# prstrive/SCGaussian

Hardware: AMD Instinct MI355X
Metric: train_iters_per_sec (higher is better)
Workload: dtype f32; 1 GPU; S2: 200000 Gaussians, 1008x756, SH degree 3, fwd+bwd per view (BASELINE configs[1] shape: LLFF-fern 3-view training, 200 k Gaussians @ 1008x756); gaussians=200000, width=1008, height=756, sh_degree=3, visible=174771, views=3, parallelism=single, ranks_seen=1, launched_by=single process, grad_bucket_bytes=0, grad_bucket_bytes_per_view=0

## Files before the change

scgaussian_amd/csrc/blend.hip:

```cpp
#include "scg_common.h"
#include "tile_sort.h"

namespace scg {

constexpr float kHalfLog2e = 0.72134752044448170f;
typedef float f32x2 __attribute__((ext_vector_type(2)));
typedef float f32x4 __attribute__((ext_vector_type(4)));

__device__ __forceinline__ bool splat_hits_rect(const float4& a, const float4& b, float x0, float y0) {
    const float dx0 = x0 - a.x, dy0 = y0 - a.y, dx1 = dx0 + 7.0f, dy1 = dy0 + 7.0f;
    const float nx = __builtin_amdgcn_fmed3f(0.0f, dx0, dx1), ny = __builtin_amdgcn_fmed3f(0.0f, dy0, dy1);
    const float cb2 = a.w + a.w;
    const float ya = __builtin_amdgcn_fmed3f(b.w * nx, dy0, dy1);
    const float qa = nx * (a.z * nx + cb2 * ya) + b.x * ya * ya;
    const float xb = __builtin_amdgcn_fmed3f(-a.w * ny * __builtin_amdgcn_rcpf(a.z), dx0, dx1);
    const float qb = ny * (b.x * ny + cb2 * xb) + a.z * xb * xb;
    return !((qa > b.z) && (qb > b.z));
}

__device__ __forceinline__ int quadrant_workgroup(int wg, int n_tiles, const uint2* __restrict__ ranges, int& quad) {
    quad = (wg >> 3) & 3;
    const int per = (n_tiles + 7) >> 3;
    const uint32_t* order = reinterpret_cast<const uint32_t*>(ranges) + 2 * (size_t)n_tiles;
    return (int)order[(wg & 7) * per + (wg >> 5)];
}

__device__ __forceinline__ void wave_sync() {
    __builtin_amdgcn_fence(__ATOMIC_ACQ_REL, "wavefront");
    __builtin_amdgcn_wave_barrier();
}

typedef const uint32_t __attribute__((address_space(3))) * LdsIds;
template <class IdList>
__device__ __forceinline__ void forward_walk(float4* s_rec, const FrameDev& f, int tile, int quad, int lane, uint2 range,
                                             IdList list,
                                             const float4* __restrict__ splats, float* __restrict__ out_color,
                                             float* __restrict__ out_depth, float* __restrict__ out_alpha,
                                             float* __restrict__ final_T, uint32_t* __restrict__ n_contrib) {
    const int tile_x = tile % f.gx, tile_y = tile / f.gx;
    const int qx0 = tile_x * kTile + (quad & 1) * 8, qy0 = tile_y * kTile + (quad >> 1) * 8;
    const int px = qx0 + (lane & 7), py = qy0 + (lane >> 3);
    const bool inside = (px < f.W) && (py < f.H);
    const float pxf = (float)px, pyf = (float)py;

    const int n = (int)(range.y - range.x);
    float T = inside ? 1.0f : -1.0f;
    int bgi0 = __builtin_amdgcn_readfirstlane(__builtin_bit_cast(int, f.bg[0]));
    int bgi1 = __builtin_amdgcn_readfirstlane(__builtin_bit_cast(int, f.bg[1]));
    int bgi2 = __builtin_amdgcn_readfirstlane(__builtin_bit_cast(int, f.bg[2]));
    asm volatile("" : "+s"(bgi0), "+s"(bgi1), "+s"(bgi2));
    f32x2 Crg = {0.f, 0.f}, Cbz = {0.f, 0.f};
    uint32_t last = 0;
    int n_blended = 0;
#ifndef SCG_FWD_TRIP_CXX
    const uint32_t lds_base = (uint32_t)reinterpret_cast<uintptr_t>(s_rec);
    const uint64_t exec_all = __builtin_amdgcn_read_exec();
#endif

    uint32_t id_next = 0;
    float4 ra, rb, rc;
    if (n > 0) {
        const uint32_t id0 = list[min(lane, n - 1)];
        id_next = list[min(kWave + lane, n - 1)];
        ra = splats[3 * (size_t)id0 + 0]; rb = splats[3 * (size_t)id0 + 1]; rc = splats[3 * (size_t)id0 + 2];
    }

    for (int base = 0; base < n; base += kWave) {
        if (__all(T < 0.0f)) break;
        const bool hit = (base + lane < n) && splat_hits_rect(ra, rb, (float)qx0, (float)qy0);
        if (hit) {
            *reinterpret_cast<float2*>(&s_rec[2 * kWave + lane]) = make_float2(ra.x, ra.y);
            s_rec[kWave + lane] = make_float4(kHalfLog2e * ra.z, 2.0f * kHalfLog2e * ra.w, kHalfLog2e * rb.x, rb.y);
            s_rec[lane] = rc;
        }
        uint64_t m = __ballot(hit);
        if (base + kWave < n) {
            ra = splats[3 * (size_t)id_next + 0]; rb = splats[3 * (size_t)id_next + 1];
            rc = splats[3 * (size_t)id_next + 2];
            id_next = list[min(base + 2 * kWave + lane, n - 1)];
        }
        wave_sync();

        n_blended += __builtin_popcountll(m);
#ifdef SCG_FWD_TRIP_CXX
        while (m) {
            const int j = __builtin_ctzll(m);
            asm("s_bitset0_b64 %0, %1" : "+s"(m) : "s"(j));
            const float2 c = *reinterpret_cast<const float2*>(&s_rec[2 * kWave + j]);
            const float4 q = s_rec[kWave + j];
            const float dx = c.x - pxf, dy = c.y - pyf;
            const float u = __builtin_fmaf(q.y, dy, q.x * dx);
            const float t = __builtin_fmaf(u, dx, (q.z * dy) * dy);
            const float alpha = fminf(kAlphaMax, q.w * __builtin_amdgcn_exp2f(-t));
            const float wgt = T * alpha;
            const float test_T = __builtin_fmaf(-T, alpha, T);
            if ((t >= 0.0f) && (alpha >= kAlphaMin)) {
                const bool contributes = test_T >= kTEps;
                const float T_prev = T;
                T = contributes ? test_T : -fabsf(T_prev);
                if (contributes) {
                    const float4 col = s_rec[j];
                    const f32x2 ww = {wgt, wgt};
                    Crg = __builtin_elementwise_fma((f32x2){col.x, col.y}, ww, Crg);
                    Cbz = __builtin_elementwise_fma((f32x2){col.z, col.w}, ww, Cbz);
                    last = (uint32_t)(base + j + 1);
                }
            }
        }
#else
        int last_j = -1;
        while (m) {
            const int j = __builtin_ctzll(m);
            asm("s_bitset0_b64 %0, %1" : "+s"(m) : "s"(j));
            asm volatile(
                "v_lshl_add_u32 v63, %[j], 4, %[lds]\n\t"
                "ds_read_b64 v[48:49], v63 offset:2048\n\t"
                "ds_read_b128 v[52:55], v63 offset:1024\n\t"
                "s_waitcnt lgkmcnt(1)\n\t"
                "v_sub_f32_e32 v48, v48, %[px]\n\t"
                "v_sub_f32_e32 v49, v49, %[py]\n\t"
                "s_waitcnt lgkmcnt(0)\n\t"
                "v_mul_f32_e32 v58, v52, v48\n\t"
                "v_mul_f32_e32 v59, v54, v49\n\t"
                "v_fmac_f32_e32 v58, v53, v49\n\t"
                "v_mul_f32_e32 v60, v59, v49\n\t"
                "v_fmac_f32_e32 v60, v58, v48\n\t"
                "v_exp_f32_e64 v56, -v60\n\t"
                "v_cmpx_le_f32_e32 vcc, 0, v60\n\t"
                "v_mul_f32_e32 v56, v55, v56\n\t"
                "v_min_f32_e32 v56, 0x3f7d70a4, v56\n\t"
                "v_cmpx_le_f32_e32 vcc, %[amin], v56\n\t"
                "v_fma_f32 v57, -%[T], v56, %[T]\n\t"
                "v_mul_f32_e32 v56, %[T], v56\n\t"
                "v_or_b32_e32 %[T], 0x80000000, %[T]\n\t"
                "v_cmpx_le_f32_e32 vcc, %[eps], v57\n\t"
                "v_mov_b32_e32 %[T], v57\n\t"
                "ds_read_b128 v[44:47], v63\n\t"
                "v_mov_b32_e32 %[lj], %[j]\n\t"
                "s_waitcnt lgkmcnt(0)\n\t"
                "v_pk_fma_f32 %[crg], v[44:45], v[56:57], %[crg] op_sel_hi:[1,0,1]\n\t"
                "v_pk_fma_f32 %[cbz], v[46:47], v[56:57], %[cbz] op_sel_hi:[1,0,1]\n\t"
                "s_mov_b64 exec, %[all]"
                : [T] "+v"(T), [crg] "+v"(Crg), [cbz] "+v"(Cbz), [lj] "+v"(last_j)
                : [j] "s"(j), [lds] "v"(lds_base), [px] "v"(pxf), [py] "v"(pyf), [amin] "s"(kAlphaMin), [eps] "s"(kTEps),
                  [all] "s"(exec_all)
                : "memory", "vcc", "v44", "v45", "v46", "v47", "v48", "v49", "v52", "v53", "v54", "v55", "v56", "v57", "v58",
                  "v59", "v60", "v63");
        }
        if (last_j >= 0) last = (uint32_t)(base + last_j + 1);
#endif
        wave_sync();
    }

    if (f.cost_out && lane == 0) atomicMax(f.cost_out + tile, (uint32_t)n_blended);
    if (inside) {
        T = fabsf(T);
        const size_t pix = (size_t)py * f.W + px;
        const size_t hw = (size_t)f.H * f.W;
        out_color[pix] = Crg[0] + T * __builtin_bit_cast(float, bgi0);
        out_color[hw + pix] = Crg[1] + T * __builtin_bit_cast(float, bgi1);
        out_color[2 * hw + pix] = Cbz[0] + T * __builtin_bit_cast(float, bgi2);
        out_depth[pix] = Cbz[1];
        out_alpha[pix] = 1.0f - T;
        if (final_T) final_T[pix] = T;
        if (n_contrib) n_contrib[pix] = last;
    }
}


__global__ __launch_bounds__(kWave) void blend_forward_kernel(FrameDev f, const uint2* __restrict__ ranges,
                                                              const uint32_t* __restrict__ point_list,
                                                              const float4* __restrict__ splats,
                                                              float* __restrict__ out_color,
                                                              float* __restrict__ out_depth,
                                                              float* __restrict__ out_alpha,
                                                              float* __restrict__ final_T,
                                                              uint32_t* __restrict__ n_contrib,
                                                              float4* __restrict__ zero_fill, uint32_t zero_vec) {
    __shared__ float4 s_rec[3 * kWave];
    if (zero_fill) {
        for (uint32_t i = blockIdx.x * kWave + threadIdx.x; i < zero_vec; i += gridDim.x * kWave)
            zero_fill[i] = make_float4(0.f, 0.f, 0.f, 0.f);
    }

    const int n_tiles = f.gx * f.gy;
    int quad;
    const int tile = quadrant_workgroup(blockIdx.x, n_tiles, ranges, quad);
    if (tile >= n_tiles) return;
    const uint2 range = ranges[tile];
    forward_walk(s_rec, f, tile, quad, (int)threadIdx.x, range, point_list + range.x, splats, out_color, out_depth, out_alpha,
                 final_T, n_contrib);
}

template <int NW>
__device__ __forceinline__ void fused_long_list_fallback(unsigned char* smem, const uint32_t* __restrict__ depth_keys,
                                                      uint32_t* __restrict__ list, int n, uint64_t* __restrict__ keys,
                                                      uint64_t* __restrict__ keys2) {
    if (!sort_long_list<NW * kWave, kFusedLongBuckets, 2>(smem, depth_keys, list, n, keys, keys2)) {
        __syncthreads();
        for (int i = threadIdx.x; i < n; i += NW * kWave) {
            const uint32_t id = list[i];
            keys[i] = ((uint64_t)depth_keys[id] << 32) | (uint64_t)id;
        }
        __syncthreads();
        bitonic_sort_asc(keys, n, true);
        __syncthreads();
        for (int i = threadIdx.x; i < n; i += NW * kWave) list[i] = (uint32_t)keys[i];
    }
}

template <int MAX_N, int CNT, int WPE, int NW = 4>
__global__ __launch_bounds__(NW * kWave) __attribute__((amdgpu_waves_per_eu(WPE, WPE))) void tile_blend_forward_kernel(
    FrameDev f, const uint2* __restrict__ ranges, uint32_t* __restrict__ point_list,
    const uint32_t* __restrict__ depth_keys, int id_bits, const float4* __restrict__ splats,
    float* __restrict__ out_color, float* __restrict__ out_depth, float* __restrict__ out_alpha,
    float* __restrict__ final_T, uint32_t* __restrict__ n_contrib, float4* __restrict__ zero_fill, uint32_t zero_vec,
    uint64_t* __restrict__ spill, uint64_t* __restrict__ spill2, const uint32_t* __restrict__ class_counts,
    int long_presorted) {
    typedef TileSortLds<NW, MAX_N, CNT> Lds;
    constexpr size_t kIdsBytes = sizeof(uint32_t) * MAX_N, kPlanesBytes = 4 * 3 * kWave * sizeof(float4);
    constexpr size_t kLdsBytes = sizeof(Lds) > kIdsBytes + kPlanesBytes ? sizeof(Lds) : kIdsBytes + kPlanesBytes;
    __shared__ __attribute__((aligned(16))) unsigned char smem[kLdsBytes];
    Lds& L = *reinterpret_cast<Lds*>(smem);
    static_assert(offsetof(Lds, id) == 0, "the sorted ids lie in front of the record planes");
    static_assert(kLdsBytes >= (2 * kFusedLongBuckets + 4 + 2 * 4) * sizeof(uint32_t), "the fallback's counters must fit");
    if (zero_fill) {
        for (uint32_t i = blockIdx.x * blockDim.x + threadIdx.x; i < zero_vec; i += gridDim.x * blockDim.x)
            zero_fill[i] = make_float4(0.f, 0.f, 0.f, 0.f);
    }
    if (f.long_out && blockIdx.x == 0 && threadIdx.x == 0) {
        f.long_out[0] = class_counts[0] + class_counts[1];
        f.long_out[1] = class_counts[3];
    }
    const int n_tiles = f.gx * f.gy, per = (n_tiles + 7) >> 3;
    const uint32_t* order = reinterpret_cast<const uint32_t*>(ranges) + 2 * (size_t)n_tiles;
    const int tile = (int)order[(blockIdx.x & 7) * per + (blockIdx.x >> 3)];
    if (tile >= n_tiles) return;
    const uint2 range = ranges[tile];
    const int n = (int)(range.y - range.x);
#ifdef SCG_PROBE_TIMELINE
    const uint32_t tp0 = (uint32_t)wall_clock64();
#endif
    const bool ids_in_lds = n >= 2 && n <= MAX_N;
    if (ids_in_lds) sort_one_tile<NW, MAX_N, CNT, true>(L, range, depth_keys, point_list, id_bits);
    else if (n > MAX_N && !long_presorted)
        fused_long_list_fallback<NW>(smem, depth_keys, point_list + range.x, n, spill + range.x, spill2 + range.x);
#ifdef SCG_PROBE_TIMELINE
    const uint32_t tp1 = (uint32_t)wall_clock64();
    uint32_t pr[6];
    for (int k = 0; k < 6; ++k) pr[k] = L.probe[k];
    __syncthreads();
#else
    if (!ids_in_lds) __syncthreads();
#endif
    const int quad = (int)threadIdx.x >> 6, lane = (int)threadIdx.x & (kWave - 1);
    if (NW > 4 && quad >= 4) return;
#ifdef SCG_PROBE_TIMELINE
    const uint32_t tp2 = (uint32_t)wall_clock64();
#endif
    float4* planes = reinterpret_cast<float4*>(smem + kIdsBytes) + quad * 3 * kWave;
    if (ids_in_lds)
        forward_walk(planes, f, tile, quad, lane, range, reinterpret_cast<LdsIds>((uintptr_t)(uint32_t)reinterpret_cast<uintptr_t>(&L.id[0])),
                     splats, out_color, out_depth, out_alpha, final_T, n_contrib);
    else
        forward_walk(planes, f, tile, quad, lane, range, point_list + range.x, splats, out_color, out_depth, out_alpha, final_T,
                     n_contrib);
#ifdef SCG_PROBE_TIMELINE
    if (f.cost_out && lane == 0) {
        uint32_t* tl = f.cost_out + n_tiles + 65792 + 32768 + ((size_t)blockIdx.x * 4 + quad) * 8;
        tl[0] = tp0; tl[1] = tp1; tl[2] = tp2; tl[3] = (uint32_t)wall_clock64(); tl[4] = (uint32_t)n; tl[5] = (uint32_t)tile;
        tl[6] = 0u; tl[7] = 0xB1E9D000u;
        if (quad == 0) {
            uint32_t* t2 = f.cost_out + n_tiles + 65792 + 32768 + ((size_t)tile_order_slots(n_tiles) * 4 + blockIdx.x) * 8;
            for (int k = 0; k < 6; ++k) t2[k] = pr[k];
            t2[6] = tp0; t2[7] = 0x50B70000u;
        }
    }
#endif
}

int launch_tile_blend_forward(const FrameDev& f, const uint32_t* ranges, uint32_t* point_list, const uint32_t* depth_keys,
                              const float* splats, float* out_color, float* out_depth, float* out_alpha,
                              float* final_T, uint32_t* n_contrib, float* dsplats_zero, void* bin_scratch, int64_t R,
                              bool long_presorted, hipStream_t stream) {
    const int n_tiles = f.gx * f.gy;
    int id_bits = 8;
    while (id_bits < 32 && (1ll << id_bits) < (long long)f.P) id_bits += 8;
    const TileBinningLayout BL = tile_binning_layout(f.P, R, n_tiles);
    uint64_t* spill = reinterpret_cast<uint64_t*>(reinterpret_cast<char*>(bin_scratch) + BL.spill);
    const bool dense = fused_max_list(R, n_tiles) == kFusedDenseMaxN;
    auto kernel = dense ? tile_blend_forward_kernel<kFusedDenseMaxN, kFusedDenseCounters, kFusedDenseWpe, kFusedDenseWaves>
                        : tile_blend_forward_kernel<kFusedMaxN, kFusedCounters, 8>;
    hipLaunchKernelGGL(kernel, dim3(tile_order_slots(n_tiles)), dim3((dense ? kFusedDenseWaves : 4) * kWave), 0, stream, f,
                       reinterpret_cast<const uint2*>(ranges), point_list, depth_keys, id_bits,
                       reinterpret_cast<const float4*>(splats), out_color, out_depth, out_alpha, final_T, n_contrib,
                       reinterpret_cast<float4*>(dsplats_zero), (uint32_t)((size_t)f.P * SCG_DSPLAT_FLOATS / 4),
                       spill, spill + R,
                       reinterpret_cast<const uint32_t*>(reinterpret_cast<char*>(bin_scratch) + BL.class_counts),
                       long_presorted ? 1 : 0);
    return check_hip(hipGetLastError(), "tile_blend_forward_kernel");
}

int launch_blend_forward(const FrameDev& f, const uint32_t* ranges, const uint32_t* point_list,
                         const float* splats, float* out_color, float* out_depth, float* out_alpha,
                         float* final_T, uint32_t* n_contrib, float* dsplats_zero, hipStream_t stream) {
    const int n_tiles = f.gx * f.gy;
    const int grid = ((n_tiles + 7) / 8) * 8 * 4;
    hipLaunchKernelGGL(blend_forward_kernel, dim3(grid), dim3(kWave), 0, stream, f,
                       reinterpret_cast<const uint2*>(ranges), point_list, reinterpret_cast<const float4*>(splats),
                       out_color, out_depth, out_alpha, final_T, n_contrib, reinterpret_cast<float4*>(dsplats_zero),
                       (uint32_t)((size_t)f.P * SCG_DSPLAT_FLOATS / 4));
    return check_hip(hipGetLastError(), "blend_forward_kernel");
}


constexpr int kSlots = 4;
constexpr int kWStride = 2 * kWave;

__device__ __forceinline__ float row_reduce10(float v0, float v1, float v2, float v3, float v4, float v5, float v6,
                                              float v7, float v8, float v9, uint64_t odd, uint64_t hi) {
    float y, t0, t1, t2, t3, t4, t5, t6, t7;
    asm("s_nop 1\n\t"
        "v_add_f32_dpp %1, %9, %9 row_shl:4 row_mask:0xf bank_mask:0x5\n\t"
        "v_add_f32_dpp %2, %11, %11 row_shl:4 row_mask:0xf bank_mask:0x5\n\t"
        "v_add_f32_dpp %3, %13, %13 row_shl:4 row_mask:0xf bank_mask:0x5\n\t"
        "v_add_f32_dpp %4, %15, %15 row_shl:4 row_mask:0xf bank_mask:0x5\n\t"
        "v_add_f32_dpp %5, %17, %17 row_shl:4 row_mask:0xf bank_mask:0x5\n\t"
        "v_add_f32_dpp %1, %10, %10 row_shr:4 row_mask:0xf bank_mask:0xa\n\t"
        "v_add_f32_dpp %2, %12, %12 row_shr:4 row_mask:0xf bank_mask:0xa\n\t"
        "v_add_f32_dpp %3, %14, %14 row_shr:4 row_mask:0xf bank_mask:0xa\n\t"
        "v_add_f32_dpp %4, %16, %16 row_shr:4 row_mask:0xf bank_mask:0xa\n\t"
        "v_add_f32_dpp %5, %18, %18 row_shr:4 row_mask:0xf bank_mask:0xa\n\t"
        "v_add_f32_dpp %6, %1, %1 row_ror:8 row_mask:0xf bank_mask:0x3\n\t"
        "v_add_f32_dpp %7, %3, %3 row_ror:8 row_mask:0xf bank_mask:0x3\n\t"
        "v_add_f32_dpp %6, %2, %2 row_ror:8 row_mask:0xf bank_mask:0xc\n\t"
        "v_add_f32_dpp %7, %4, %4 row_ror:8 row_mask:0xf bank_mask:0xc\n\t"
        "v_add_f32_dpp %8, %5, %5 row_ror:8 row_mask:0xf bank_mask:0xf\n\t"
        "v_cndmask_b32 %1, %6, %7, %19\n\t"
        "v_cndmask_b32 %2, %7, %6, %19\n\t"
        "v_add_f32_dpp %3, %8, %8 quad_perm:[1,0,3,2] row_mask:0xf bank_mask:0xf\n\t"
        "s_nop 0\n\t"
        "v_add_f32_dpp %4, %2, %1 quad_perm:[1,0,3,2] row_mask:0xf bank_mask:0xf\n\t"
        "v_cndmask_b32 %5, %4, %3, %20\n\t"
        "v_cndmask_b32 %1, %3, %4, %20\n\t"
        "s_nop 1\n\t"
        "v_add_f32_dpp %0, %1, %5 quad_perm:[2,3,0,1] row_mask:0xf bank_mask:0xf"
        : "=&v"(y), "=&v"(t0), "=&v"(t1), "=&v"(t2), "=&v"(t3), "=&v"(t4), "=&v"(t5), "=&v"(t6), "=&v"(t7)
        : "v"(v0), "v"(v1), "v"(v2), "v"(v3), "v"(v4), "v"(v5), "v"(v6), "v"(v7), "v"(v8), "v"(v9), "s"(odd), "s"(hi));
    return y;
}

struct BwdLds {
    float4 a[kWave];
    float4 b[kWave];
    float4 c[kWave];
    __attribute__((aligned(16))) float w[kSlots * kWStride];
};

struct BwdPixel {
    float T, behind, dC0, dC1, dC2, dD, dA;
    uint32_t last;
};

__device__ __forceinline__ uint32_t top_chunk_index(int end) {
    return (uint32_t)min(((end - 1) / kWave) * kWave + (kWave - 1 - (int)threadIdx.x), end - 1);
}
__device__ __forceinline__ int backward_walk(BwdLds& L, const FrameDev& f, int tile, int quad, int first, int end,
                                              BwdPixel px, uint32_t list_begin, uint32_t id_top,
                                              const uint32_t* __restrict__ point_list,
                                              const float4* __restrict__ splats, float* __restrict__ dsplats) {
    const int lane = threadIdx.x;
    const int tile_x = tile % f.gx, tile_y = tile / f.gx;
    const int qx0 = tile_x * kTile + (quad & 1) * 8, qy0 = tile_y * kTile + (quad >> 1) * 8;
    const float pxf = (float)(qx0 + (lane & 7)), pyf = (float)(qy0 + (lane >> 3));
    float T = px.T, behind = px.behind;
    const float dC0 = px.dC0, dC1 = px.dC1, dC2 = px.dC2, dD = px.dD, dA = px.dA;
    const uint32_t last = px.last;

    const int row = lane >> 4, grp = lane & 15;
    float4 fc[4];
    {
        float4* tmp = reinterpret_cast<float4*>(L.w);
        __syncthreads();
        tmp[lane] = make_float4(dC0, dC1, dC2, dD);
        __syncthreads();
#pragma unroll
        for (int i = 0; i < 4; ++i) fc[i] = tmp[grp + 16 * i];
        __syncthreads();
    }
    const float gx_pix = (float)(qx0 + (grp & 7)), gy_pix = (float)(qy0 + (grp >> 3));
    float* w_store = L.w + 2 * lane;
#ifdef SCG_FWD_TRIP_CXX
    const float* w_load = L.w + row * kWStride + 2 * grp;
#else
    const uint32_t lds_wl = (uint32_t)reinterpret_cast<uintptr_t>(L.w + row * kWStride + 2 * grp);
    typedef const float __attribute__((address_space(3))) * LdsFloats;
#define w_load reinterpret_cast<LdsFloats>((uintptr_t)lds_wl)
#endif
    const int bank = (lane >> 2) & 3, qq_ = lane & 3;
    int out_slot = -1;
    if (qq_ < 2 || (qq_ == 2 && bank < 2)) {
        const int quantity = (qq_ == 0) ? bank : (qq_ == 1) ? 4 + bank : 8 + bank;
        out_slot = (quantity < 7) ? quantity : quantity + 1;
    }
    const uint32_t out_bytes = (uint32_t)(out_slot < 0 ? 0 : out_slot) * 4u;

    int slot = 0;
    float my_x = 0.f, my_y = 0.f;
    uint32_t my_id = 0;

    const uint64_t out_lanes = __ballot(out_slot >= 0);
    const uint64_t lanes_all = __builtin_amdgcn_read_exec();
    uint64_t odd_lanes = 0xAAAAAAAAAAAAAAAAull, hi_lanes = 0xCCCCCCCCCCCCCCCCull;
    asm volatile("" : "+s"(odd_lanes), "+s"(hi_lanes));
    auto flush = [&](int rows, float dx, float dy0) {
        __builtin_amdgcn_fence(__ATOMIC_ACQ_REL, "wavefront");
        __builtin_amdgcn_wave_barrier();
#ifdef SCG_FWD_TRIP_CXX
        const float2 qw0 = *reinterpret_cast<const float2*>(w_load);
#else
        const float2 qw0 = make_float2(w_load[0], w_load[1]);
#endif
        const float qy0 = qw0.x * dy0;
        float Sq = qw0.x, Sy = qy0, Syy = qy0 * dy0, Rr = qw0.y * fc[0].x, Gg = qw0.y * fc[0].y, Bb = qw0.y * fc[0].z,
              Dz = qw0.y * fc[0].w;
#pragma unroll
        for (int i = 1; i < 4; ++i) {
#ifdef SCG_FWD_TRIP_CXX
            const float2 qw = *reinterpret_cast<const float2*>(w_load + 32 * i);
#else
            const float2 qw = make_float2(w_load[32 * i], w_load[32 * i + 1]);
#endif
            const float dy = dy0 - (float)(2 * i);
            const float qy = qw.x * dy;
            Sq += qw.x;
            Sy += qy;
            Syy = __builtin_fmaf(qy, dy, Syy);
            Rr = __builtin_fmaf(qw.y, fc[i].x, Rr);
            Gg = __builtin_fmaf(qw.y, fc[i].y, Gg);
            Bb = __builtin_fmaf(qw.y, fc[i].z, Bb);
            Dz = __builtin_fmaf(qw.y, fc[i].w, Dz);
        }
        const float Sx = dx * Sq, Sxx = dx * Sx, Sxy = dx * Sy;
        const float sum = row_reduce10(Sx, Sy, Dz, Sq,
                                       Sxx, Sxy, Syy, Rr,
                                       Gg, Bb, odd_lanes, hi_lanes);
        const uint32_t rec = my_id * (uint32_t)(SCG_DSPLAT_FLOATS * 4) + out_bytes;
        const uint64_t lanes = (rows >= kSlots) ? out_lanes : (out_lanes & ((1ull << (16 * rows)) - 1ull));
        asm volatile("s_mov_b64 exec, %[lanes]\n\t"
                     "global_atomic_add_f32 %[off], %[val], %[base]\n\t"
                     "s_mov_b64 exec, %[all]"
                     :: [lanes] "s"(lanes), [off] "v"(rec), [val] "v"(sum), [base] "s"(dsplats), [all] "s"(lanes_all)
                     : "memory");
        __builtin_amdgcn_fence(__ATOMIC_ACQ_REL, "wavefront");
        __builtin_amdgcn_wave_barrier();
    };

    float amax_s;
    asm volatile("s_mov_b32 %0, 0x3f7d70a4" : "=s"(amax_s));
    const int chunk_bot = first / kWave;
    uint32_t id = id_top;
    int n_trips = 0;
#ifdef SCG_FWD_TRIP_CXX
    float* w_ptr = w_store;
#else
    static_assert(offsetof(BwdLds, b) == 1024 && offsetof(BwdLds, c) == 2048 && kWStride * sizeof(float) == 512,
                  "the hand-written walk addresses the planes with immediate offsets");
    const uint32_t lds_rec = (uint32_t)reinterpret_cast<uintptr_t>(&L.a[0]);
    const uint32_t lds_w = (uint32_t)reinterpret_cast<uintptr_t>(w_store);
    const uint64_t row0 = 0x000000000000FFFFull, row1 = 0x00000000FFFF0000ull, row2 = 0x0000FFFF00000000ull,
                   row3 = 0xFFFF000000000000ull;
    typedef float f32x16 __attribute__((ext_vector_type(16)));
    const f32x16 fcv = {fc[0].x, fc[0].y, fc[0].z, fc[0].w, fc[1].x, fc[1].y, fc[1].z, fc[1].w,
                        fc[2].x, fc[2].y, fc[2].z, fc[2].w, fc[3].x, fc[3].y, fc[3].z, fc[3].w};
    const f32x4 dCv = {dC0, dC1, dC2, dD};
#endif
    for (int chunk = (end - 1) / kWave; chunk >= chunk_bot; --chunk) {
        const int base = chunk * kWave;
        const int k = base + (kWave - 1 - lane);
#ifdef SCG_FWD_TRIP_CXX
        const int first_j = base + (kWave - 1) - (int)last;
#else
        const int first_j = max(base + (kWave - 1) - (int)last, -1);
#endif
        const float4 a = splats[3 * (size_t)id + 0];
        const float4 b = splats[3 * (size_t)id + 1];
        const float4 c_rec = splats[3 * (size_t)id + 2];
        uint32_t id_next = id;
        if (chunk > chunk_bot) id_next = point_list[list_begin + (uint32_t)(k - kWave)];
        const bool hit = (k < end) && splat_hits_rect(a, b, (float)qx0, (float)qy0);
        if (hit) {
            L.a[lane] = make_float4(a.x, a.y, kHalfLog2e * a.z, 2.0f * kHalfLog2e * a.w);
            L.b[lane] = make_float4(kHalfLog2e * b.x, b.y, __builtin_bit_cast(float, id), 0.f);
            L.c[lane] = c_rec;
        }
        id = id_next;
        uint64_t m = __ballot(hit);
        n_trips += __builtin_popcountll(m);
        __builtin_amdgcn_s_waitcnt(0x0F70);
        __syncthreads();

#ifdef SCG_FWD_TRIP_CXX
        while (m) {
            const int j = __builtin_ctzll(m);
            asm("s_bitset0_b64 %0, %1" : "+s"(m) : "s"(j));
            const float4 a = L.a[j];
            const float4 b = L.b[j];
            const float4 c = L.c[j];
            asm("" ::"v"(b.w));
            const float dx = a.x - pxf, dy = a.y - pyf;
            float u = a.z * dx;
            asm("" : "+v"(u));
            u = __builtin_fmaf(a.w, dy, u);
            const float t = __builtin_fmaf(u, dx, (b.x * dy) * dy);
            const float oG = b.y * __builtin_amdgcn_exp2f(-t);
            const bool ok = (j > first_j) && (t >= 0.0f) && (oG >= kAlphaMin);
            if (__ballot(ok) == 0ull) continue;

            const float q0 = ok ? oG : 0.0f;
            const float alpha = __builtin_amdgcn_fmed3f(q0, 0.0f, amax_s);
            const float one_m = 1.0f - alpha;
            T *= __builtin_amdgcn_rcpf(one_m);
            const float d = __builtin_fmaf(c.x, dC0, __builtin_fmaf(c.y, dC1, __builtin_fmaf(c.z, dC2, __builtin_fmaf(c.w, dD, dA))));
            const float q = q0 * ((d - behind) * T);
            behind *= one_m;
            asm("" : "+v"(behind));
            behind = __builtin_fmaf(alpha, d, behind);
            const float wgt = alpha * T;
            *reinterpret_cast<float2*>(w_ptr) = make_float2(q, wgt);
            w_ptr += kWStride;
            const bool mine = (row == slot);
            my_x = mine ? a.x : my_x;
            my_y = mine ? a.y : my_y;
            my_id = mine ? __builtin_bit_cast(uint32_t, b.z) : my_id;
            if (++slot == kSlots) {
                flush(kSlots, my_x - gx_pix, my_y - gy_pix);
                slot = 0;
                w_ptr = w_store;
            }
        }
#else
#define SCG_BWD_ROW(K, NEXT)                                                                                                 \
            ".Ltrip" #K "_%=:\n\t"                                                                                         \
            "s_ff1_i32_b64 s90, %[m]\n\t"                           \
            "s_bitset0_b64 %[m], s90\n\t"                                                                                 \
            "v_lshl_add_u32 v60, s90, 4, %[rec]\n\t"                                                                      \
            "ds_read_b128 v[48:51], v60\n\t"                                                                               \
            "ds_read_b128 v[52:55], v60 offset:1024\n\t"                                                                   \
            "ds_read_b128 v[44:47], v60 offset:2048\n\t"                                                                   \
            "v_mov_b32_e32 v58, 0\n\t"                                                                                     \
            "v_mov_b32_e32 v59, 0\n\t"                                                                                     \
            "v_cmpx_gt_i32_e32 vcc, s90, %[fj]\n\t"                 \
            "s_waitcnt lgkmcnt(2)\n\t"                                                                                     \
            "v_sub_f32_e32 v56, v48, %[px]\n\t"                                                                            \
            "v_sub_f32_e32 v57, v49, %[py]\n\t"                                                                            \
            "v_mul_f32_e32 v50, v56, v50\n\t"                                                                  \
            "s_waitcnt lgkmcnt(1)\n\t"                                                                                     \
            "v_mul_f32_e32 v52, v57, v52\n\t"                                                                  \
            "v_fmac_f32_e32 v50, v51, v57\n\t"                                                  \
            "v_mul_f32_e32 v52, v57, v52\n\t"                                                                \
            "v_fmac_f32_e32 v52, v50, v56\n\t"                                                            \
            "v_exp_f32_e64 v51, -v52\n\t"                                                                                  \
            "v_cmpx_le_f32_e32 vcc, 0, v52\n\t"                                                  \
            "v_mul_f32_e32 v51, v53, v51\n\t"                                                               \
            "v_cmpx_le_f32_e32 vcc, 0x3b808081, v51\n\t"                                \
            "s_cbranch_execz .Lnone" #K "_%=\n\t"                                                                          \
            "v_min_f32_e32 v50, 0x3f7d70a4, v51\n\t"                                     \
            "v_sub_f32_e32 v52, 1.0, v50\n\t"                                                       \
            "v_rcp_f32_e32 v56, v52\n\t"                                                                                   \
            "s_waitcnt lgkmcnt(0)\n\t"                                                                                     \
            "v_fma_f32 v57, v47, v27, %[dA]\n\t"                   \
            "v_fmac_f32_e32 v57, v46, v26\n\t"                                                                          \
            "v_fmac_f32_e32 v57, v45, v25\n\t"                                                                          \
            "v_fmac_f32_e32 v57, v44, v24\n\t"                                                                          \
            "v_mul_f32_e32 %[T], %[T], v56\n\t"                                  \
            "v_sub_f32_e32 v58, v57, %[bh]\n\t"                                                                            \
            "v_mul_f32_e32 v58, v58, %[T]\n\t"                                                                             \
            "v_mul_f32_e32 v58, v51, v58\n\t"                                                 \
            "v_mul_f32_e32 %[bh], %[bh], v52\n\t"                               \
            "v_fmac_f32_e32 %[bh], v50, v57\n\t"                                                                           \
            "v_mul_f32_e32 v59, v50, %[T]\n\t"                                                            \
            "s_mov_b64 exec, %[row" #K "]\n\t"                               \
            "v_sub_f32_e32 %[mdx], v48, %[px]\n\t"                     \
            "v_sub_f32_e32 %[mdy], v49, %[gy]\n\t"                                                                        \
            "v_mov_b32_e32 %[mi], v54\n\t"                                                                                 \
            "s_mov_b64 exec, -1\n\t"                                          \
            "ds_write_b64 %[wst], v[58:59] offset:" NEXT "\n\t"
#define SCG_BWD_NONE(K)                                                                                                      \
            ".Lnone" #K "_%=:\n\t"                                                                                         \
            "s_mov_b64 exec, -1\n\t"                                                                                   \
            "s_cmp_lt_i32 s90, 0\n\t"                                                                                     \
            "s_cbranch_scc0 .Ltrip" #K "_%=\n\t"                                                                           \
            "s_mov_b32 %[slot], " #K "\n\t"                                                                                \
            "s_branch .Lend_%=\n\t"
        {
            asm volatile(
                "s_cmp_eq_u32 %[slot], 0\n\t"
                "s_cbranch_scc1 .Ltrip0_%=\n\t"
                "s_cmp_eq_u32 %[slot], 1\n\t"
                "s_cbranch_scc1 .Ltrip1_%=\n\t"
                "s_cmp_eq_u32 %[slot], 2\n\t"
                "s_cbranch_scc1 .Ltrip2_%=\n\t"
                "s_branch .Ltrip3_%=\n\t"
                SCG_BWD_NONE(0)
                SCG_BWD_NONE(1)
                SCG_BWD_NONE(2)
                SCG_BWD_NONE(3)
                SCG_BWD_ROW(0, "0")
                SCG_BWD_ROW(1, "512")
                SCG_BWD_ROW(2, "1024")
                SCG_BWD_ROW(3, "1536")
                "ds_read2_b64 v[44:47], %[wld] offset1:16\n\t"
                "ds_read2_b64 v[48:51], %[wld] offset0:32 offset1:48\n\t"
                "v_add_f32_e32 v52, -2.0, %[mdy]\n\t"
                "v_add_f32_e32 v53, -4.0, %[mdy]\n\t"
                "v_add_f32_e32 v54, 0xc0c00000, %[mdy]\n\t"
                "s_waitcnt lgkmcnt(1)\n\t"
                "v_mul_f32_e32 v55, v44, %[mdy]\n\t"
                "v_mul_f32_e32 v57, v45, v28\n\t"
                "v_mul_f32_e32 v58, v45, v29\n\t"
                "v_mul_f32_e32 v59, v45, v30\n\t"
                "v_mul_f32_e32 v60, v45, v31\n\t"
                "v_mul_f32_e32 v56, v55, %[mdy]\n\t"
                "v_mul_f32_e32 v61, v46, v52\n\t"
                "v_add_f32_e32 v44, v44, v46\n\t"
                "v_fmac_f32_e32 v57, v47, v32\n\t"
                "v_fmac_f32_e32 v58, v47, v33\n\t"
                "v_fmac_f32_e32 v59, v47, v34\n\t"
                "v_fmac_f32_e32 v60, v47, v35\n\t"
                "v_add_f32_e32 v55, v55, v61\n\t"
                "v_fmac_f32_e32 v56, v61, v52\n\t"
                "s_waitcnt lgkmcnt(0)\n\t"
                "v_mul_f32_e32 v61, v48, v53\n\t"
                "v_add_f32_e32 v44, v44, v48\n\t"
                "v_fmac_f32_e32 v57, v49, v36\n\t"
                "v_fmac_f32_e32 v58, v49, v37\n\t"
                "v_fmac_f32_e32 v59, v49, v38\n\t"
                "v_fmac_f32_e32 v60, v49, v39\n\t"
                "v_add_f32_e32 v55, v55, v61\n\t"
                "v_fmac_f32_e32 v56, v61, v53\n\t"
                "v_mul_f32_e32 v61, v50, v54\n\t"
                "v_add_f32_e32 v44, v44, v50\n\t"
                "v_fmac_f32_e32 v57, v51, v40\n\t"
                "v_fmac_f32_e32 v58, v51, v41\n\t"
                "v_fmac_f32_e32 v59, v51, v42\n\t"
                "v_fmac_f32_e32 v60, v51, v43\n\t"
                "v_add_f32_e32 v55, v55, v61\n\t"
                "v_fmac_f32_e32 v56, v61, v54\n\t"
                "v_mul_f32_e32 v45, %[mdx], v44\n\t"
                "v_mul_f32_e32 v47, %[mdx], v55\n\t"
                "v_mul_f32_e32 v46, %[mdx], v45\n\t"
                "s_nop 1\n\t"
                "v_add_f32_dpp v48, v45, v45 row_shl:4 row_mask:0xf bank_mask:0x5\n\t"
                "v_add_f32_dpp v49, v60, v60 row_shl:4 row_mask:0xf bank_mask:0x5\n\t"
                "v_add_f32_dpp v50, v46, v46 row_shl:4 row_mask:0xf bank_mask:0x5\n\t"
                "v_add_f32_dpp v51, v56, v56 row_shl:4 row_mask:0xf bank_mask:0x5\n\t"
                "v_add_f32_dpp v52, v58, v58 row_shl:4 row_mask:0xf bank_mask:0x5\n\t"
                "v_add_f32_dpp v48, v55, v55 row_shr:4 row_mask:0xf bank_mask:0xa\n\t"
                "v_add_f32_dpp v49, v44, v44 row_shr:4 row_mask:0xf bank_mask:0xa\n\t"
                "v_add_f32_dpp v50, v47, v47 row_shr:4 row_mask:0xf bank_mask:0xa\n\t"
                "v_add_f32_dpp v51, v57, v57 row_shr:4 row_mask:0xf bank_mask:0xa\n\t"
                "v_add_f32_dpp v52, v59, v59 row_shr:4 row_mask:0xf bank_mask:0xa\n\t"
                "v_add_f32_dpp v53, v48, v48 row_ror:8 row_mask:0xf bank_mask:0x3\n\t"
                "v_add_f32_dpp v54, v50, v50 row_ror:8 row_mask:0xf bank_mask:0x3\n\t"
                "v_add_f32_dpp v53, v49, v49 row_ror:8 row_mask:0xf bank_mask:0xc\n\t"
                "v_add_f32_dpp v54, v51, v51 row_ror:8 row_mask:0xf bank_mask:0xc\n\t"
                "v_add_f32_dpp v61, v52, v52 row_ror:8 row_mask:0xf bank_mask:0xf\n\t"
                "v_cndmask_b32_e64 v48, v53, v54, %[odd]\n\t"
                "v_cndmask_b32_e64 v49, v54, v53, %[odd]\n\t"
                "v_add_f32_dpp v50, v61, v61 quad_perm:[1,0,3,2] row_mask:0xf bank_mask:0xf\n\t"
                "s_nop 0\n\t"
                "v_add_f32_dpp v51, v49, v48 quad_perm:[1,0,3,2] row_mask:0xf bank_mask:0xf\n\t"
                "v_cndmask_b32_e64 v52, v51, v50, %[hi]\n\t"
                "v_cndmask_b32_e64 v48, v50, v51, %[hi]\n\t"
                "v_lshl_add_u32 v44, %[mi], 6, %[ob]\n\t"
                "s_nop 0\n\t"
                "v_add_f32_dpp v45, v48, v52 quad_perm:[2,3,0,1] row_mask:0xf bank_mask:0xf\n\t"
                "s_mov_b64 exec, %[lanes]\n\t"
                "global_atomic_add_f32 v44, v45, %[base]\n\t"
                "s_mov_b64 exec, -1\n\t"
                "s_branch .Ltrip0_%=\n\t"
                ".Lend_%=:\n\t"
                "s_waitcnt lgkmcnt(0)"
                : [m] "+s"(m), [slot] "+s"(slot), [T] "+v"(T), [bh] "+v"(behind), [mdx] "+v"(my_x), [mdy] "+v"(my_y),
                  [mi] "+v"(my_id)
                : [rec] "v"(lds_rec), [wst] "v"(lds_w), [wld] "v"(lds_wl), [fj] "v"(first_j), [px] "v"(pxf), [py] "v"(pyf),
                  [gy] "v"(gy_pix), [ob] "v"(out_bytes), [dA] "v"(dA), "{v[24:27]}"(dCv), "{v[28:43]}"(fcv),
                  [row0] "s"(row0), [row1] "s"(row1), [row2] "s"(row2), [row3] "s"(row3), [lanes] "s"(out_lanes),
                  [odd] "s"(odd_lanes), [hi] "s"(hi_lanes), [base] "s"(dsplats)
                : "memory", "vcc", "scc", "s90", "s91", "v44", "v45", "v46", "v47", "v48", "v49", "v50", "v51", "v52", "v53",
                  "v54", "v55", "v56", "v57", "v58", "v59", "v60", "v61");
        }
#undef SCG_BWD_NONE
#undef SCG_BWD_ROW
#endif
        __syncthreads();
    }
#ifdef SCG_FWD_TRIP_CXX
    if (slot > 0) flush(slot, my_x - gx_pix, my_y - gy_pix);
#else
    if (slot > 0) flush(slot, my_x, my_y);
#undef w_load
#endif
    return n_trips;
}

__device__ __forceinline__ BwdPixel load_pixel_final(const FrameDev& f, int px, int py, const float* __restrict__ final_T,
                                                     const uint32_t* __restrict__ n_contrib,
                                                     const float* __restrict__ dL_dcolor, const float* __restrict__ dL_ddepth,
                                                     const float* __restrict__ dL_dalpha) {
    BwdPixel s;
    s.T = 1.0f; s.dC0 = s.dC1 = s.dC2 = s.dD = s.dA = 0.f; s.last = 0;
    if ((px < f.W) && (py < f.H)) {
        const size_t pix = (size_t)py * f.W + px;
        const size_t hw = (size_t)f.H * f.W;
        s.T = final_T[pix];
        s.last = n_contrib[pix];
        s.dC0 = dL_dcolor[pix]; s.dC1 = dL_dcolor[hw + pix]; s.dC2 = dL_dcolor[2 * hw + pix];
        if (dL_ddepth) s.dD = dL_ddepth[pix];
        if (dL_dalpha) s.dA = dL_dalpha[pix];
    }
    s.behind = f.bg[0] * s.dC0 + f.bg[1] * s.dC1 + f.bg[2] * s.dC2;
    return s;
}

#ifdef SCG_BWD_WAVES
#define SCG_BWD_OCCUPANCY __attribute__((amdgpu_waves_per_eu(SCG_BWD_WAVES, SCG_BWD_WAVES)))
#else
#define SCG_BWD_OCCUPANCY
#endif
__global__ __launch_bounds__(kWave) SCG_BWD_OCCUPANCY void blend_backward_kernel(
    FrameDev f, const uint2* __restrict__ ranges, const uint32_t* __restrict__ point_list,
    const float4* __restrict__ splats, const float* __restrict__ final_T, const uint32_t* __restrict__ n_contrib,
    const float* __restrict__ dL_dcolor, const float* __restrict__ dL_ddepth, const float* __restrict__ dL_dalpha,
    float* __restrict__ dsplats) {
    __shared__ BwdLds L;
    const int n_tiles = f.gx * f.gy;
    const int slots = tile_order_slots(n_tiles);
    const uint32_t* order_q = reinterpret_cast<const uint32_t*>(ranges) + 2 * (size_t)n_tiles + slots;
    const uint32_t entry = order_q[(size_t)(blockIdx.x & 7) * (4 * (slots >> 3)) + (blockIdx.x >> 3)];
    const int tile = (int)(entry >> 2), quad = (int)(entry & 3u);
    if (tile >= n_tiles) return;
    const int lane = threadIdx.x;
    const int px = (tile % f.gx) * kTile + (quad & 1) * 8 + (lane & 7), py = (tile / f.gx) * kTile + (quad >> 1) * 8 + (lane >> 3);
    const uint2 range = ranges[tile];
    const int n = (int)(range.y - range.x);
    const BwdPixel s = load_pixel_final(f, px, py, final_T, n_contrib, dL_dcolor, dL_ddepth, dL_dalpha);
    uint32_t mx = s.last;
#pragma unroll
    for (int off = 32; off > 0; off >>= 1) mx = max(mx, (uint32_t)__shfl_down((int)mx, off, kWave));
    const int limit = min(n, __builtin_amdgcn_readfirstlane((int)mx));
#ifdef SCG_PROBE_TIMELINE
    const uint32_t tp0 = (uint32_t)wall_clock64();
#endif
    if (limit <= 0) {
        if (f.bcost_out && lane == 0) f.bcost_out[4 * tile + quad] = 0u;
        return;
    }
    const int trips = backward_walk(L, f, tile, quad, 0, limit, s, range.x, point_list[range.x + top_chunk_index(limit)],
                                    point_list, splats, dsplats);
    if (f.bcost_out && lane == 0) f.bcost_out[4 * tile + quad] = (uint32_t)trips;
#ifdef SCG_PROBE_TIMELINE
    if (f.cost_out && lane == 0) {
        uint32_t* tl = f.cost_out + n_tiles + 65792 + 32768 + (size_t)(n_tiles + 8) * 40 + (size_t)blockIdx.x * 4;
        tl[0] = tp0; tl[1] = (uint32_t)wall_clock64(); tl[2] = ((uint32_t)min(trips, 65535) << 16) | (uint32_t)min(limit, 65535);
        tl[3] = 0xBAC00000u | (uint32_t)(4 * tile + quad);
    }
#endif
}

int launch_blend_backward(const FrameDev& f, const uint32_t* ranges, const uint32_t* point_list,
                          const float* splats, const float* final_T, const uint32_t* n_contrib,
                          const float* dL_dcolor, const float* dL_ddepth, const float* dL_dalpha,
                          float* dsplats, bool dsplats_prezeroed, hipStream_t stream, hipEvent_t started, hipEvent_t done) {
    if (!dsplats_prezeroed) {
        const int rc = check_hip(hipMemsetAsync(dsplats, 0, (size_t)f.P * SCG_DSPLAT_FLOATS * sizeof(float), stream),
                                 "dsplats memset");
        if (rc) return rc;
    }
    const int n_tiles = f.gx * f.gy;
    const int grid = ((n_tiles + 7) / 8) * 8 * 4;
    if (started || done) {
        hipExtLaunchKernelGGL(blend_backward_kernel, dim3(grid), dim3(kWave), 0u, stream, started, done, 0u, f,
                              reinterpret_cast<const uint2*>(ranges), point_list, reinterpret_cast<const float4*>(splats),
                              final_T, n_contrib, dL_dcolor, dL_ddepth, dL_dalpha, dsplats);
    } else {
        hipLaunchKernelGGL(blend_backward_kernel, dim3(grid), dim3(kWave), 0, stream, f,
                           reinterpret_cast<const uint2*>(ranges), point_list, reinterpret_cast<const float4*>(splats),
                           final_T, n_contrib, dL_dcolor, dL_ddepth, dL_dalpha, dsplats);
    }
    return check_hip(hipGetLastError(), "blend_backward_kernel");
}

}
```

Before: 4306 iters/s.

## Track kept splat record indices in SGPRs instead of per-row masked VGPR copies

The backward blending walk no longer copies the x, y and id of each accumulated splat into VGPRs under per-row exec masks. It records the LDS record index in packed scalar registers and reloads the record at flush time. Records still pending when a chunk ends are copied into extra LDS slots appended to the record arrays, which shifts the plane offsets. The weight-buffer zeroing is folded into an exchange-on-read at flush, removing two moves per row. This trims VALU and exec-switch work in the hot loop, at the cost of extra LDS traffic and a more intricate carry-over path.

```diff
diff --git a/scgaussian_amd/csrc/blend.hip b/scgaussian_amd/csrc/blend.hip
--- a/scgaussian_amd/csrc/blend.hip
+++ b/scgaussian_amd/csrc/blend.hip
@@ -350,9 +350,10 @@
     return y;
 }
 
+constexpr int kRecs = kWave + kSlots;
 struct BwdLds {
-    float4 a[kWave];
-    float4 b[kWave];
+    float4 a[kRecs];
+    float4 b[kRecs];
     float4 c[kWave];
     __attribute__((aligned(16))) float w[kSlots * kWStride];
 };
@@ -390,6 +391,10 @@
     }
     const float gx_pix = (float)(qx0 + (grp & 7)), gy_pix = (float)(qy0 + (grp >> 3));
     float* w_store = L.w + 2 * lane;
+#ifndef SCG_FWD_TRIP_CXX
+#pragma unroll
+    for (int r = 0; r < kSlots; ++r) *reinterpret_cast<float2*>(w_store + r * kWStride) = make_float2(0.f, 0.f);
+#endif
 #ifdef SCG_FWD_TRIP_CXX
     const float* w_load = L.w + row * kWStride + 2 * grp;
 #else
@@ -406,14 +411,19 @@
     const uint32_t out_bytes = (uint32_t)(out_slot < 0 ? 0 : out_slot) * 4u;
 
     int slot = 0;
+#ifdef SCG_FWD_TRIP_CXX
     float my_x = 0.f, my_y = 0.f;
     uint32_t my_id = 0;
+#else
+    uint32_t keep01 = 0, keep23 = 0;
+    const uint32_t keep_shift = (uint32_t)(16 * (row & 1) + 8 * (row >> 1));
+#endif
 
     const uint64_t out_lanes = __ballot(out_slot >= 0);
     const uint64_t lanes_all = __builtin_amdgcn_read_exec();
     uint64_t odd_lanes = 0xAAAAAAAAAAAAAAAAull, hi_lanes = 0xCCCCCCCCCCCCCCCCull;
     asm volatile("" : "+s"(odd_lanes), "+s"(hi_lanes));
-    auto flush = [&](int rows, float dx, float dy0) {
+    auto flush = [&](int rows, float dx, float dy0, uint32_t my_id) {
         __builtin_amdgcn_fence(__ATOMIC_ACQ_REL, "wavefront");
         __builtin_amdgcn_wave_barrier();
 #ifdef SCG_FWD_TRIP_CXX
@@ -464,12 +474,13 @@
 #ifdef SCG_FWD_TRIP_CXX
     float* w_ptr = w_store;
 #else
-    static_assert(offsetof(BwdLds, b) == 1024 && offsetof(BwdLds, c) == 2048 && kWStride * sizeof(float) == 512,
+    static_assert(offsetof(BwdLds, b) == 1088 && offsetof(BwdLds, c) == 2176 && kWStride * sizeof(float) == 512,
                   "the hand-written walk addresses the planes with immediate offsets");
+    static_assert(kRecs < 256 && sizeof(BwdLds) <= 5376, "record entries fit a byte; LDS per wave <= 5.25 KiB");
     const uint32_t lds_rec = (uint32_t)reinterpret_cast<uintptr_t>(&L.a[0]);
     const uint32_t lds_w = (uint32_t)reinterpret_cast<uintptr_t>(w_store);
-    const uint64_t row0 = 0x000000000000FFFFull, row1 = 0x00000000FFFF0000ull, row2 = 0x0000FFFF00000000ull,
-                   row3 = 0xFFFF000000000000ull;
+    uint64_t zero2 = 0;
+    asm volatile("" : "+v"(zero2));
     typedef float f32x16 __attribute__((ext_vector_type(16)));
     const f32x16 fcv = {fc[0].x, fc[0].y, fc[0].z, fc[0].w, fc[1].x, fc[1].y, fc[1].z, fc[1].w,
                         fc[2].x, fc[2].y, fc[2].z, fc[2].w, fc[3].x, fc[3].y, fc[3].z, fc[3].w};
@@ -534,22 +545,20 @@
             my_y = mine ? a.y : my_y;
             my_id = mine ? __builtin_bit_cast(uint32_t, b.z) : my_id;
             if (++slot == kSlots) {
-                flush(kSlots, my_x - gx_pix, my_y - gy_pix);
+                flush(kSlots, my_x - gx_pix, my_y - gy_pix, my_id);
                 slot = 0;
                 w_ptr = w_store;
             }
         }
 #else
-#define SCG_BWD_ROW(K, NEXT)                                                                                                 \
+#define SCG_BWD_ROW(K, NEXT, KEEP)                                                                                           \
             ".Ltrip" #K "_%=:\n\t"                                                                                         \
             "s_ff1_i32_b64 s90, %[m]\n\t"                           \
             "s_bitset0_b64 %[m], s90\n\t"                                                                                 \
             "v_lshl_add_u32 v60, s90, 4, %[rec]\n\t"                                                                      \
             "ds_read_b128 v[48:51], v60\n\t"                                                                               \
-            "ds_read_b128 v[52:55], v60 offset:1024\n\t"                                                                   \
-            "ds_read_b128 v[44:47], v60 offset:2048\n\t"                                                                   \
-            "v_mov_b32_e32 v58, 0\n\t"                                                                                     \
-            "v_mov_b32_e32 v59, 0\n\t"                                                                                     \
+            "ds_read_b128 v[52:55], v60 offset:1088\n\t"                                                                   \
+            "ds_read_b128 v[44:47], v60 offset:2176\n\t"                                                                   \
             "v_cmpx_gt_i32_e32 vcc, s90, %[fj]\n\t"                 \
             "s_waitcnt lgkmcnt(2)\n\t"                                                                                     \
             "v_sub_f32_e32 v56, v48, %[px]\n\t"                                                                            \
@@ -580,12 +589,9 @@
             "v_mul_f32_e32 %[bh], %[bh], v52\n\t"                               \
             "v_fmac_f32_e32 %[bh], v50, v57\n\t"                                                                           \
             "v_mul_f32_e32 v59, v50, %[T]\n\t"                                                            \
-            "s_mov_b64 exec, %[row" #K "]\n\t"                               \
-            "v_sub_f32_e32 %[mdx], v48, %[px]\n\t"                     \
-            "v_sub_f32_e32 %[mdy], v49, %[gy]\n\t"                                                                        \
-            "v_mov_b32_e32 %[mi], v54\n\t"                                                                                 \
-            "s_mov_b64 exec, -1\n\t"                                          \
-            "ds_write_b64 %[wst], v[58:59] offset:" NEXT "\n\t"
+            KEEP "\n\t"                                                                       \
+            "ds_write_b64 %[wst], v[58:59] offset:" NEXT "\n\t"                  \
+            "s_mov_b64 exec, -1\n\t"
 #define SCG_BWD_NONE(K)                                                                                                      \
             ".Lnone" #K "_%=:\n\t"                                                                                         \
             "s_mov_b64 exec, -1\n\t"                                                                                   \
@@ -606,50 +612,59 @@
                 SCG_BWD_NONE(1)
                 SCG_BWD_NONE(2)
                 SCG_BWD_NONE(3)
-                SCG_BWD_ROW(0, "0")
-                SCG_BWD_ROW(1, "512")
-                SCG_BWD_ROW(2, "1024")
-                SCG_BWD_ROW(3, "1536")
-                "ds_read2_b64 v[44:47], %[wld] offset1:16\n\t"
-                "ds_read2_b64 v[48:51], %[wld] offset0:32 offset1:48\n\t"
-                "v_add_f32_e32 v52, -2.0, %[mdy]\n\t"
-                "v_add_f32_e32 v53, -4.0, %[mdy]\n\t"
-                "v_add_f32_e32 v54, 0xc0c00000, %[mdy]\n\t"
+                SCG_BWD_ROW(0, "0", "s_mov_b32 %[k01], s90")
+                SCG_BWD_ROW(1, "512", "s_pack_ll_b32_b16 %[k01], %[k01], s90")
+                SCG_BWD_ROW(2, "1024", "s_mov_b32 %[k23], s90")
+                SCG_BWD_ROW(3, "1536", "s_pack_ll_b32_b16 %[k23], %[k23], s90")
+                "s_lshl_b32 s91, %[k23], 8\n\t"
+                "s_or_b32 s91, s91, %[k01]\n\t"
+                "v_bfe_u32 v52, s91, %[ksh], 8\n\t"
+                "v_lshl_add_u32 v52, v52, 4, %[rec]\n\t"
+                "ds_read2_b64 v[52:55], v52 offset1:137\n\t"
+                "ds_wrxchg2_rtn_b64 v[44:47], %[wld], %[z], %[z] offset1:16\n\t"
+                "ds_wrxchg2_rtn_b64 v[48:51], %[wld], %[z], %[z] offset0:32 offset1:48\n\t"
+                "s_waitcnt lgkmcnt(2)\n\t"
+                "v_sub_f32_e32 v52, v52, %[px]\n\t"
+                "v_sub_f32_e32 v53, v53, %[gy]\n\t"
+                "v_lshl_add_u32 v54, v54, 6, %[ob]\n\t"
+                "v_add_f32_e32 v62, -2.0, v53\n\t"
                 "s_waitcnt lgkmcnt(1)\n\t"
-                "v_mul_f32_e32 v55, v44, %[mdy]\n\t"
+                "v_mul_f32_e32 v55, v44, v53\n\t"
                 "v_mul_f32_e32 v57, v45, v28\n\t"
                 "v_mul_f32_e32 v58, v45, v29\n\t"
                 "v_mul_f32_e32 v59, v45, v30\n\t"
                 "v_mul_f32_e32 v60, v45, v31\n\t"
-                "v_mul_f32_e32 v56, v55, %[mdy]\n\t"
-                "v_mul_f32_e32 v61, v46, v52\n\t"
+                "v_mul_f32_e32 v56, v55, v53\n\t"
+                "v_mul_f32_e32 v61, v46, v62\n\t"
                 "v_add_f32_e32 v44, v44, v46\n\t"
                 "v_fmac_f32_e32 v57, v47, v32\n\t"
                 "v_fmac_f32_e32 v58, v47, v33\n\t"
                 "v_fmac_f32_e32 v59, v47, v34\n\t"
                 "v_fmac_f32_e32 v60, v47, v35\n\t"
                 "v_add_f32_e32 v55, v55, v61\n\t"
-                "v_fmac_f32_e32 v56, v61, v52\n\t"
+                "v_fmac_f32_e32 v56, v61, v62\n\t"
+                "v_add_f32_e32 v62, -4.0, v53\n\t"
                 "s_waitcnt lgkmcnt(0)\n\t"
-                "v_mul_f32_e32 v61, v48, v53\n\t"
+                "v_mul_f32_e32 v61, v48, v62\n\t"
                 "v_add_f32_e32 v44, v44, v48\n\t"
                 "v_fmac_f32_e32 v57, v49, v36\n\t"
                 "v_fmac_f32_e32 v58, v49, v37\n\t"
                 "v_fmac_f32_e32 v59, v49, v38\n\t"
                 "v_fmac_f32_e32 v60, v49, v39\n\t"
                 "v_add_f32_e32 v55, v55, v61\n\t"
-                "v_fmac_f32_e32 v56, v61, v53\n\t"
-                "v_mul_f32_e32 v61, v50, v54\n\t"
+                "v_fmac_f32_e32 v56, v61, v62\n\t"
+                "v_add_f32_e32 v62, 0xc0c00000, v53\n\t"
+                "v_mul_f32_e32 v61, v50, v62\n\t"
                 "v_add_f32_e32 v44, v44, v50\n\t"
                 "v_fmac_f32_e32 v57, v51, v40\n\t"
                 "v_fmac_f32_e32 v58, v51, v41\n\t"
                 "v_fmac_f32_e32 v59, v51, v42\n\t"
                 "v_fmac_f32_e32 v60, v51, v43\n\t"
                 "v_add_f32_e32 v55, v55, v61\n\t"
-                "v_fmac_f32_e32 v56, v61, v54\n\t"
-                "v_mul_f32_e32 v45, %[mdx], v44\n\t"
-                "v_mul_f32_e32 v47, %[mdx], v55\n\t"
-                "v_mul_f32_e32 v46, %[mdx], v45\n\t"
+                "v_fmac_f32_e32 v56, v61, v62\n\t"
+                "v_mul_f32_e32 v45, v52, v44\n\t"
+                "v_mul_f32_e32 v47, v52, v55\n\t"
+                "v_mul_f32_e32 v46, v52, v45\n\t"
                 "s_nop 1\n\t"
                 "v_add_f32_dpp v48, v45, v45 row_shl:4 row_mask:0xf bank_mask:0x5\n\t"
                 "v_add_f32_dpp v49, v60, v60 row_shl:4 row_mask:0xf bank_mask:0x5\n\t"
@@ -662,44 +677,57 @@
                 "v_add_f32_dpp v51, v57, v57 row_shr:4 row_mask:0xf bank_mask:0xa\n\t"
                 "v_add_f32_dpp v52, v59, v59 row_shr:4 row_mask:0xf bank_mask:0xa\n\t"
                 "v_add_f32_dpp v53, v48, v48 row_ror:8 row_mask:0xf bank_mask:0x3\n\t"
-                "v_add_f32_dpp v54, v50, v50 row_ror:8 row_mask:0xf bank_mask:0x3\n\t"
+                "v_add_f32_dpp v62, v50, v50 row_ror:8 row_mask:0xf bank_mask:0x3\n\t"
                 "v_add_f32_dpp v53, v49, v49 row_ror:8 row_mask:0xf bank_mask:0xc\n\t"
-                "v_add_f32_dpp v54, v51, v51 row_ror:8 row_mask:0xf bank_mask:0xc\n\t"
+                "v_add_f32_dpp v62, v51, v51 row_ror:8 row_mask:0xf bank_mask:0xc\n\t"
                 "v_add_f32_dpp v61, v52, v52 row_ror:8 row_mask:0xf bank_mask:0xf\n\t"
-                "v_cndmask_b32_e64 v48, v53, v54, %[odd]\n\t"
-                "v_cndmask_b32_e64 v49, v54, v53, %[odd]\n\t"
+                "v_cndmask_b32_e64 v48, v53, v62, %[odd]\n\t"
+                "v_cndmask_b32_e64 v49, v62, v53, %[odd]\n\t"
                 "v_add_f32_dpp v50, v61, v61 quad_perm:[1,0,3,2] row_mask:0xf bank_mask:0xf\n\t"
                 "s_nop 0\n\t"
                 "v_add_f32_dpp v51, v49, v48 quad_perm:[1,0,3,2] row_mask:0xf bank_mask:0xf\n\t"
                 "v_cndmask_b32_e64 v52, v51, v50, %[hi]\n\t"
                 "v_cndmask_b32_e64 v48, v50, v51, %[hi]\n\t"
-                "v_lshl_add_u32 v44, %[mi], 6, %[ob]\n\t"
-                "s_nop 0\n\t"
+                "s_nop 1\n\t"
                 "v_add_f32_dpp v45, v48, v52 quad_perm:[2,3,0,1] row_mask:0xf bank_mask:0xf\n\t"
                 "s_mov_b64 exec, %[lanes]\n\t"
-                "global_atomic_add_f32 v44, v45, %[base]\n\t"
+                "global_atomic_add_f32 v54, v45, %[base]\n\t"
                 "s_mov_b64 exec, -1\n\t"
                 "s_branch .Ltrip0_%=\n\t"
                 ".Lend_%=:\n\t"
                 "s_waitcnt lgkmcnt(0)"
-                : [m] "+s"(m), [slot] "+s"(slot), [T] "+v"(T), [bh] "+v"(behind), [mdx] "+v"(my_x), [mdy] "+v"(my_y),
-                  [mi] "+v"(my_id)
+                : [m] "+s"(m), [slot] "+s"(slot), [T] "+v"(T), [bh] "+v"(behind), [k01] "+s"(keep01), [k23] "+s"(keep23)
                 : [rec] "v"(lds_rec), [wst] "v"(lds_w), [wld] "v"(lds_wl), [fj] "v"(first_j), [px] "v"(pxf), [py] "v"(pyf),
-                  [gy] "v"(gy_pix), [ob] "v"(out_bytes), [dA] "v"(dA), "{v[24:27]}"(dCv), "{v[28:43]}"(fcv),
-                  [row0] "s"(row0), [row1] "s"(row1), [row2] "s"(row2), [row3] "s"(row3), [lanes] "s"(out_lanes),
-                  [odd] "s"(odd_lanes), [hi] "s"(hi_lanes), [base] "s"(dsplats)
+                  [gy] "v"(gy_pix), [ob] "v"(out_bytes), [ksh] "v"(keep_shift), [z] "v"(zero2), [dA] "v"(dA),
+                  "{v[24:27]}"(dCv), "{v[28:43]}"(fcv), [lanes] "s"(out_lanes), [odd] "s"(odd_lanes), [hi] "s"(hi_lanes),
+                  [base] "s"(dsplats)
                 : "memory", "vcc", "scc", "s90", "s91", "v44", "v45", "v46", "v47", "v48", "v49", "v50", "v51", "v52", "v53",
-                  "v54", "v55", "v56", "v57", "v58", "v59", "v60", "v61");
+                  "v54", "v55", "v56", "v57", "v58", "v59", "v60", "v61", "v62");
         }
 #undef SCG_BWD_NONE
 #undef SCG_BWD_ROW
+        if (slot > 0 && chunk > chunk_bot) {
+            if (lane < slot) {
+                const uint32_t e = ((lane < 2 ? keep01 : keep23) >> (16 * (lane & 1))) & 0xFFFFu;
+                const float4 a = L.a[e];
+                const float id_bits = L.b[e].z;
+                L.a[kWave + lane] = a;
+                L.b[kWave + lane].z = id_bits;
+            }
+            keep01 = (uint32_t)kWave | ((uint32_t)(kWave + 1) << 16);
+            keep23 = (uint32_t)(kWave + 2) | ((uint32_t)(kWave + 3) << 16);
+        }
 #endif
         __syncthreads();
     }
 #ifdef SCG_FWD_TRIP_CXX
-    if (slot > 0) flush(slot, my_x - gx_pix, my_y - gy_pix);
-#else
-    if (slot > 0) flush(slot, my_x, my_y);
+    if (slot > 0) flush(slot, my_x - gx_pix, my_y - gy_pix, my_id);
+#else
+    if (slot > 0) {
+        const uint32_t e = (((keep23 << 8) | keep01) >> keep_shift) & 0xFFu;
+        const float4 a = L.a[e];
+        flush(slot, a.x - gx_pix, a.y - gy_pix, __builtin_bit_cast(uint32_t, L.b[e].z));
+    }
 #undef w_load
 #endif
     return n_trips;
```

Result: no change. 4329 iters/s, median of 6 (+0.5%).
